# Doubiiu/ToonCrafter

Measured on AMD Instinct MI355X. Metric: interpolated frames/sec, 512x320x16f DDIM-50, higher is better.
Workload: dtype bf16; 1 GPU; ToonCrafter_512 320x512x16f ddim_steps=50 CFG 7.5 bf16, 1 clip per GPU (BASELINE.json configs[1]); sampler + 16f decode + 14f re-decode + splice; a different clip every step; parallelism=dp1 (independent clips, one RCCL gather)

## Files before the change

tooncrafter_amd/csrc/attention.hip:

```cpp
#include "attn_tile64.h"
#include "gemm_common.h"

#include <stdlib.h>

namespace {

constexpr int KT = 64;
constexpr int K_STRIDE = 144;
constexpr int VT_STRIDE = 136;
constexpr int K_BYTES = KT * K_STRIDE;
constexpr int VT_BYTES = 64 * VT_STRIDE;

__global__ __launch_bounds__(256) void attn_d64_kernel(const TcAttnParams p) {
  __shared__ __attribute__((aligned(16))) char smem[K_BYTES + VT_BYTES];
  char* ks = smem;
  char* vts = smem + K_BYTES;

  const int tid = threadIdx.x, lane = tid & 63, wave = tid >> 6;
  const int l31 = lane & 31, half = lane >> 5;
  const int b = blockIdx.z, h = blockIdx.y;
  const int kvb = b / p.kv_bdiv;
  const bf16_t* qb = reinterpret_cast<const bf16_t*>(p.q) + (int64_t)b * p.q_sb + h * 64;
  const bf16_t* kb = reinterpret_cast<const bf16_t*>(p.k) + (int64_t)kvb * p.k_sb + h * 64;
  const bf16_t* vb = reinterpret_cast<const bf16_t*>(p.v) + (int64_t)kvb * p.v_sb + h * 64;
  bf16_t* ob = reinterpret_cast<bf16_t*>(p.o) + (int64_t)b * p.o_sb + h * 64;

  const int q_row = blockIdx.x * 128 + wave * 32 + l31;
  bf16x8 qf[4];
  tc_tile64_load_q(qf, qb, q_row, p.lq, p.q_ss, half);

  const float c = p.scale * 1.4426950408889634f;
  float m_run = -1e30f, l_run = 0.f;
  f32x16 oacc[2];
#pragma unroll
  for (int d = 0; d < 2; ++d)
#pragma unroll
    for (int r = 0; r < 16; ++r) oacc[d][r] = 0.f;

  u32x4 kreg[2], vreg[2];
  const u32x4 zero4 = {0u, 0u, 0u, 0u};
  auto load_kv = [&](int kt) {
    const int key0 = kt * KT;
#pragma unroll
    for (int it = 0; it < 2; ++it) {
      const int idx = tid + it * 256;
      const int key = idx & 63, dch = idx >> 6;
      const int gk = key0 + key;
      const int gkc = gk < p.lk ? gk : p.lk - 1;
      kreg[it] = *reinterpret_cast<const u32x4*>(kb + (int64_t)gkc * p.k_ss + dch * 8);
      vreg[it] = *reinterpret_cast<const u32x4*>(vb + (int64_t)gkc * p.v_ss + dch * 8);
    }
  };
  auto store_kv = [&](int kt) {
    const int key0 = kt * KT;
    uint16_t* vt = reinterpret_cast<uint16_t*>(vts);
#pragma unroll
    for (int it = 0; it < 2; ++it) {
      const int idx = tid + it * 256;
      const int key = idx & 63, dch = idx >> 6;
      const bool ok = key0 + key < p.lk;
      const u32x4 kv4 = ok ? kreg[it] : zero4;
      const u32x4 vv4 = ok ? vreg[it] : zero4;
      *reinterpret_cast<u32x4*>(ks + key * K_STRIDE + dch * 16) = kv4;
#pragma unroll
      for (int e = 0; e < 4; ++e) {
        vt[(dch * 8 + 2 * e) * (VT_STRIDE / 2) + key] = (uint16_t)(vv4[e] & 0xffffu);
        vt[(dch * 8 + 2 * e + 1) * (VT_STRIDE / 2) + key] = (uint16_t)(vv4[e] >> 16);
      }
    }
  };

  const int n_tiles = (p.lk + KT - 1) / KT;
  load_kv(0);
  for (int kt = 0; kt < n_tiles; ++kt) {
    const int key0 = kt * KT;
    __syncthreads();
    store_kv(kt);
    __syncthreads();
    if (kt + 1 < n_tiles) load_kv(kt + 1);

    f32x16 st[2];
    const f32x16 zero16 = {0.f, 0.f, 0.f, 0.f, 0.f, 0.f, 0.f, 0.f, 0.f, 0.f, 0.f, 0.f, 0.f, 0.f, 0.f, 0.f};
#pragma unroll
    for (int kbk = 0; kbk < 2; ++kbk) {
#pragma unroll
      for (int kk = 0; kk < 4; ++kk) {
        const bf16x8 kf = *reinterpret_cast<const bf16x8*>(ks + (kbk * 32 + l31) * K_STRIDE + kk * 32 + half * 16);
        st[kbk] = __builtin_amdgcn_mfma_f32_32x32x16_bf16(kf, qf[kk], kk == 0 ? zero16 : st[kbk], 0, 0, 0);
      }
    }
    tc_tile64_mask(st, key0, p.lk, half, -1e30f);
    tc_tile64_softmax(st, c, m_run, l_run, oacc);

#pragma unroll
    for (int kbk = 0; kbk < 2; ++kbk)
#pragma unroll
      for (int s = 0; s < 2; ++s) {
        const bf16x8 pf = tc_tile64_pack_p(st[kbk], s);
#pragma unroll
        for (int d = 0; d < 2; ++d) {
          const char* vrow = vts + (d * 32 + l31) * VT_STRIDE + (kbk * 32 + 16 * s + 4 * half) * 2;
          const u32x2 lo = *reinterpret_cast<const u32x2*>(vrow);
          const u32x2 hi = *reinterpret_cast<const u32x2*>(vrow + 16);
          u32x4 vv = {lo[0], lo[1], hi[0], hi[1]};
          oacc[d] = __builtin_amdgcn_mfma_f32_32x32x16_bf16(__builtin_bit_cast(bf16x8, vv), pf, oacc[d], 0, 0, 0);
        }
      }
  }

  if (q_row < p.lq) tc_tile64_store(oacc, l_run, ob + (int64_t)q_row * p.o_ss, half, p.accumulate);
}

constexpr int KD_TILE = KT * 128;
constexpr int DMA_STAGE = 2 * KD_TILE;

__device__ __forceinline__ u32x2 lds_read_tr16_b64(const char* p) {
  typedef short s16x4 __attribute__((ext_vector_type(4)));
  const s16x4 v = __builtin_amdgcn_ds_read_tr16_b64_v4i16((__attribute__((address_space(3))) s16x4*)(p));
  return __builtin_bit_cast(u32x2, v);
}

template <bool DUAL>
__global__ __launch_bounds__(256) void attn_d64_dma_kernel(const TcAttnParams p) {
  __shared__ __attribute__((aligned(1024))) char smem[2 * DMA_STAGE];

  const int tid = threadIdx.x, lane = tid & 63, wave = tid >> 6;
  const int wave_u = __builtin_amdgcn_readfirstlane(wave);
  const int l31 = lane & 31, half = lane >> 5;
  const int b = blockIdx.z, h = blockIdx.y;
  const bf16_t* qb = reinterpret_cast<const bf16_t*>(p.q) + (int64_t)b * p.q_sb + h * 64;
  bf16_t* ob = reinterpret_cast<bf16_t*>(p.o) + (int64_t)b * p.o_sb + h * 64;

  const int q_row = blockIdx.x * 128 + wave * 32 + l31;
  bf16x8 qf[4];
  tc_tile64_load_q(qf, qb, q_row, p.lq, p.q_ss, half);

  int k_off[4];
#pragma unroll
  for (int kk = 0; kk < 4; ++kk) k_off[kk] = l31 * 128 + (((kk * 2 + half) ^ ((l31 >> 1) & 7)) << 4);
  const int lg = lane & 15;
  int v_off[2];
#pragma unroll
  for (int d0 = 0; d0 < 2; ++d0) {
    const int vrow = lg >> 2;
    const int col = d0 * 32 + 16 * ((lane >> 4) & 1) + 4 * (lg & 3);
    const int chunk = (col >> 3) ^ (((vrow >> 1) & 1) << 2);
    v_off[d0] = vrow * 128 + chunk * 16 + (col & 7) * 2;
  }

  const float c = p.scale * 1.4426950408889634f;
  float m_run = -1e30f, l_run = 0.f;
  f32x16 oacc[2];
#pragma unroll
  for (int d = 0; d < 2; ++d)
#pragma unroll
    for (int r = 0; r < 16; ++r) oacc[d][r] = 0.f;
  const int prow = lane >> 3;

  auto run_stream = [&](const bf16_t* kb, const bf16_t* vb, const int lk, const int k_ss, const int v_ss) {
    const tc_rsrc_t k_rsrc = make_rsrc(kb, ((int64_t)(lk - 1) * k_ss + 64) * 2);
    const tc_rsrc_t v_rsrc = make_rsrc(vb, ((int64_t)(lk - 1) * v_ss + 64) * 2);
    uint32_t k_voff[2], v_voff[2];
    int piece_row[2];
#pragma unroll
    for (int i = 0; i < 2; ++i) {
      const int row = (wave + 4 * i) * 8 + prow;
      piece_row[i] = row;
      const int kchunk = (lane & 7) ^ ((row >> 1) & 7);
      const int vchunk = (lane & 7) ^ (((row >> 1) & 1) << 2);
      k_voff[i] = (uint32_t)(row * k_ss * 2 + kchunk * 16);
      v_voff[i] = (uint32_t)(row * v_ss * 2 + vchunk * 16);
    }
    auto dma_tile = [&](int kt, int stage) {
      const int key0 = kt * KT;
      char* sk = smem + stage * DMA_STAGE + wave_u * 1024;
      char* sv = sk + KD_TILE;
#pragma unroll
      for (int i = 0; i < 2; ++i) {
        const uint32_t dead = (key0 + piece_row[i] < lk) ? 0u : TC_OOB;
        glds16(k_rsrc, sk + i * 4096, k_voff[i] | dead, (uint32_t)key0 * (uint32_t)k_ss * 2u);
        glds16(v_rsrc, sv + i * 4096, v_voff[i] | dead, (uint32_t)key0 * (uint32_t)v_ss * 2u);
      }
    };

    const int n_tiles = (lk + KT - 1) / KT;
    dma_tile(0, 0);
    for (int kt = 0; kt < n_tiles; ++kt) {
      const int key0 = kt * KT;
      asm volatile("s_waitcnt vmcnt(0)" ::: "memory");
      __syncthreads();
      if (kt + 1 < n_tiles) dma_tile(kt + 1, (kt + 1) & 1);
      const char* ks = smem + (kt & 1) * DMA_STAGE;
      const char* vs = ks + KD_TILE;

      f32x16 st[2];
      const f32x16 zero16 = {0.f, 0.f, 0.f, 0.f, 0.f, 0.f, 0.f, 0.f, 0.f, 0.f, 0.f, 0.f, 0.f, 0.f, 0.f, 0.f};
#pragma unroll
      for (int kbk = 0; kbk < 2; ++kbk) {
#pragma unroll
        for (int kk = 0; kk < 4; ++kk) {
          const bf16x8 kf = *reinterpret_cast<const bf16x8*>(ks + kbk * 32 * 128 + k_off[kk]);
          st[kbk] = __builtin_amdgcn_mfma_f32_32x32x16_bf16(kf, qf[kk], kk == 0 ? zero16 : st[kbk], 0, 0, 0);
        }
      }
      tc_tile64_mask(st, key0, lk, half, -1e30f);
      tc_tile64_softmax(st, c, m_run, l_run, oacc);

#pragma unroll
      for (int kbk = 0; kbk < 2; ++kbk)
#pragma unroll
        for (int s = 0; s < 2; ++s) {
          const bf16x8 pf = tc_tile64_pack_p(st[kbk], s);
          const int kbase = (kbk * 32 + 16 * s + 4 * half) * 128;
#pragma unroll
          for (int d = 0; d < 2; ++d) {
            const u32x2 lo = lds_read_tr16_b64(vs + kbase + v_off[d]);
            const u32x2 hi = lds_read_tr16_b64(vs + kbase + 8 * 128 + v_off[d]);
            u32x4 vv = {lo[0], lo[1], hi[0], hi[1]};
            oacc[d] = __builtin_amdgcn_mfma_f32_32x32x16_bf16(__builtin_bit_cast(bf16x8, vv), pf, oacc[d], 0, 0, 0);
          }
        }
    }
  };

  {
    const int kvb = b / p.kv_bdiv;
    run_stream(reinterpret_cast<const bf16_t*>(p.k) + (int64_t)kvb * p.k_sb + h * 64,
               reinterpret_cast<const bf16_t*>(p.v) + (int64_t)kvb * p.v_sb + h * 64, p.lk, p.k_ss, p.v_ss);
  }
  f32x16 o1[2];
  if (DUAL) {
    const float inv1 = 1.0f / l_run;
#pragma unroll
    for (int d = 0; d < 2; ++d)
#pragma unroll
      for (int r = 0; r < 16; ++r) { o1[d][r] = oacc[d][r] * inv1; oacc[d][r] = 0.f; }
    m_run = -1e30f;
    l_run = 0.f;
    __syncthreads();
    const int kvb2 = b / p.kv2_bdiv;
    run_stream(reinterpret_cast<const bf16_t*>(p.k2) + (int64_t)kvb2 * p.k2_sb + h * 64,
               reinterpret_cast<const bf16_t*>(p.v2) + (int64_t)kvb2 * p.v2_sb + h * 64, p.lk2, p.k2_ss, p.v2_ss);
  }

  if (q_row < p.lq) tc_tile64_store<DUAL>(oacc, o1, l_run, ob + (int64_t)q_row * p.o_ss, half, p.accumulate);
}

__global__ __launch_bounds__(256) void attn_temporal_kernel(const bf16_t* __restrict__ qkv, bf16_t* __restrict__ out,
                                                           int nb, int t_len, int hw, int heads, float scale) {
  __shared__ float kv_s[4][2][16][64 + 4];
  const int lane = threadIdx.x & 63, wave = threadIdx.x >> 6;
  const int64_t seq = (int64_t)blockIdx.x * 4 + wave;
  const int64_t total = (int64_t)nb * hw * heads;
  const bool active = seq < total;
  const int64_t sq = active ? seq : total - 1;
  const int hd = (int)(sq % heads);
  const int64_t bp = sq / heads;
  const int px = (int)(bp % hw);
  const int bb = (int)(bp / hw);
  const int C = heads * 64;
  const int ld = 3 * C;
  const int64_t row0 = ((int64_t)bb * t_len) * hw + px;

#pragma unroll
  for (int it = 0; it < 2; ++it) {
    const int idx = lane + it * 64;
    const int fr = idx >> 3, ch = idx & 7;
    float kf[8], vf[8];
    if (fr < t_len) {
      const bf16_t* rp = qkv + (row0 + (int64_t)fr * hw) * ld + hd * 64 + ch * 8;
      unpack8(*reinterpret_cast<const u32x4*>(rp + C), kf);
      unpack8(*reinterpret_cast<const u32x4*>(rp + 2 * C), vf);
    } else {
#pragma unroll
      for (int e = 0; e < 8; ++e) { kf[e] = 0.f; vf[e] = 0.f; }
    }
#pragma unroll
// ... 38 lines not shown
#pragma unroll
  for (int j = 0; j < 16; ++j) {
    const float pj = s[j] * inv;
#pragma unroll
    for (int e = 0; e < 16; ++e) o[e] += pj * kv_s[wave][1][j][quarter * 16 + e];
  }
  if (active && qi < t_len) {
    bf16_t* op = out + (row0 + (int64_t)qi * hw) * C + hd * 64 + quarter * 16;
    *reinterpret_cast<u32x4*>(op) = pack8(o);
    *reinterpret_cast<u32x4*>(op + 8) = pack8(o + 8);
  }
}

}

extern "C" int tc_attn_d64(const TcAttnParams* pp, void* stream) {
  if (!pp) return TC_EINVAL;
  const TcAttnParams& p = *pp;
  if (!p.q || !p.k || !p.v || !p.o) return TC_EINVAL;
  if (p.batch <= 0 || p.heads <= 0 || p.lq <= 0 || p.lk <= 0 || p.kv_bdiv <= 0) return TC_EINVAL;
  if (!tc_tile64_aligned(p.q, p.q_ss, p.q_sb) || !tc_tile64_aligned(p.k, p.k_ss, p.k_sb) ||
      !tc_tile64_aligned(p.v, p.v_ss, p.v_sb) || !tc_tile64_aligned(p.o, p.o_ss, p.o_sb))
    return TC_EALIGN;
  if (p.heads > 65535 || p.batch > 65535) return TC_ESHAPE;
  const bool dual = p.k2 != nullptr;
  if (dual) {
    if (!p.v2 || p.lk2 <= 0 || p.kv2_bdiv <= 0) return TC_EINVAL;
    if (!tc_tile64_aligned(p.k2, p.k2_ss, p.k2_sb) || !tc_tile64_aligned(p.v2, p.v2_ss, p.v2_sb)) return TC_EALIGN;
  }
  dim3 grid((p.lq + 127) / 128, p.heads, p.batch), block(256);
  static const bool use_reg = [] { const char* e = getenv("TC_ATTN_STAGE"); return e && e[0] == 'r'; }();
  const bool fits = (int64_t)p.lk * p.k_ss * 2 < 0x7fffff00LL && (int64_t)p.lk * p.v_ss * 2 < 0x7fffff00LL &&
                    p.k_ss >= 64 && p.v_ss >= 64;
  if (dual) {
    const bool fits2 = (int64_t)p.lk2 * p.k2_ss * 2 < 0x7fffff00LL && (int64_t)p.lk2 * p.v2_ss * 2 < 0x7fffff00LL &&
                       p.k2_ss >= 64 && p.v2_ss >= 64;
    if (!fits || !fits2) return TC_ESHAPE;
    hipLaunchKernelGGL(attn_d64_dma_kernel<true>, grid, block, 0, reinterpret_cast<hipStream_t>(stream), p);
  } else if (!use_reg && fits) {
    hipLaunchKernelGGL(attn_d64_dma_kernel<false>, grid, block, 0, reinterpret_cast<hipStream_t>(stream), p);
  } else {
    hipLaunchKernelGGL(attn_d64_kernel, grid, block, 0, reinterpret_cast<hipStream_t>(stream), p);
  }
  TC_LAUNCH_CHECK();
  return TC_OK;
}

extern "C" int tc_attn_temporal(const tc_bf16* qkv, tc_bf16* out, int32_t b, int32_t t, int32_t hw,
                                int32_t heads, float scale, void* stream) {
  if (!qkv || !out || b <= 0 || t <= 0 || hw <= 0 || heads <= 0) return TC_EINVAL;
  if (t > TC_TEMPORAL_MAX_FRAMES) return TC_ESHAPE;
  if (!tc_aligned16(qkv) || !tc_aligned16(out)) return TC_EALIGN;
  if (t > 16)
    return attn_temporal_long_launch(reinterpret_cast<const bf16_t*>(qkv), reinterpret_cast<bf16_t*>(out), b, t, hw, heads,
                                     scale, reinterpret_cast<hipStream_t>(stream));
  const int64_t total = (int64_t)b * hw * heads;
  const int64_t nblk = (total + 3) / 4;
  if (nblk > 0x7fffffffLL) return TC_ESHAPE;
  hipLaunchKernelGGL(attn_temporal_kernel, dim3((unsigned)nblk), dim3(256), 0, reinterpret_cast<hipStream_t>(stream),
                     reinterpret_cast<const bf16_t*>(qkv), reinterpret_cast<bf16_t*>(out), b, t, hw, heads, scale);
  TC_LAUNCH_CHECK();
  return TC_OK;
}
```

tooncrafter_amd/csrc/attn_tile64.h:

```cpp
#pragma once
#include "common.h"

namespace {

__device__ __forceinline__ void tc_tile64_load_q(bf16x8 (&qf)[4], const bf16_t* qb, int q_row, int lq, int q_ss, int half) {
  const int q_ld = q_row < lq ? q_row : lq - 1;
#pragma unroll
  for (int kk = 0; kk < 4; ++kk) qf[kk] = *reinterpret_cast<const bf16x8*>(qb + (int64_t)q_ld * q_ss + kk * 16 + half * 8);
}

template <class S>
__device__ __forceinline__ void tc_tile64_mask(S (&s)[2], int key0, int lk, int half, float masked) {
  if (key0 + 64 <= lk) return;
#pragma unroll
  for (int kbk = 0; kbk < 2; ++kbk)
#pragma unroll
    for (int r = 0; r < 16; ++r) {
      const int key = key0 + kbk * 32 + (r & 3) + 8 * (r >> 2) + 4 * half;
      s[kbk][r] = key < lk ? s[kbk][r] : masked;
    }
}

__device__ __forceinline__ void tc_tile64_raise_max(float m_new, float& m_run, float& l_run, f32x16 (&oacc)[2]) {
  if (!__all(m_new == m_run)) {
// ... 5 lines not shown
      for (int r = 0; r < 16; ++r) oacc[d][r] *= alpha;
    m_run = m_new;
  }
}

__device__ __forceinline__ void tc_tile64_softmax(f32x16 (&st)[2], float c, float& m_run, float& l_run, f32x16 (&oacc)[2]) {
  float mx = st[0][0];
#pragma unroll
  for (int kbk = 0; kbk < 2; ++kbk)
#pragma unroll
    for (int r = 0; r < 16; ++r) mx = fmaxf(mx, st[kbk][r]);
  mx = fmaxf(mx, __shfl_xor(mx, 32, 64));
  tc_tile64_raise_max(fmaxf(m_run, mx * c), m_run, l_run, oacc);
  float rs = 0.f;
#pragma unroll
  for (int kbk = 0; kbk < 2; ++kbk)
#pragma unroll
    for (int r = 0; r < 16; ++r) {
      const float pv = fast_exp2(fmaf(st[kbk][r], c, -m_run));
      st[kbk][r] = pv;
      rs += pv;
    }
  rs += __shfl_xor(rs, 32, 64);
  l_run += rs;
}

__device__ __forceinline__ bf16x8 tc_tile64_pack_p(const f32x16& st, int s) {
  bf16x8 pf;
#pragma unroll
  for (int j = 0; j < 8; ++j) pf[j] = (bf16_t)st[8 * s + j];
  return pf;
}

template <bool DUAL>
__device__ __forceinline__ void tc_tile64_store(const f32x16 (&oacc)[2], const f32x16 (&o1)[2], float l_run, bf16_t* orow,
                                                int half, bool accumulate) {
  const float inv = 1.0f / l_run;
#pragma unroll
  for (int d = 0; d < 2; ++d)
#pragma unroll
    for (int g = 0; g < 4; ++g) {
      float x0 = oacc[d][4 * g + 0] * inv, x1 = oacc[d][4 * g + 1] * inv;
      float x2 = oacc[d][4 * g + 2] * inv, x3 = oacc[d][4 * g + 3] * inv;
      if (DUAL) { x0 += o1[d][4 * g + 0]; x1 += o1[d][4 * g + 1]; x2 += o1[d][4 * g + 2]; x3 += o1[d][4 * g + 3]; }
      u32x2* dst = reinterpret_cast<u32x2*>(orow + d * 32 + 8 * g + 4 * half);
      if (accumulate) {
        const u32x2 old = *dst;
        x0 += __uint_as_float(old[0] << 16);
        x1 += __uint_as_float(old[0] & 0xffff0000u);
        x2 += __uint_as_float(old[1] << 16);
        x3 += __uint_as_float(old[1] & 0xffff0000u);
      }
      const u32x2 out = {pack2(x0, x1), pack2(x2, x3)};
      *dst = out;
    }
}
__device__ __forceinline__ void tc_tile64_store(const f32x16 (&oacc)[2], float l_run, bf16_t* orow, int half, bool accumulate) {
  tc_tile64_store<false>(oacc,  oacc, l_run, orow, half, accumulate);
}

inline bool tc_tile64_aligned(const void* p, int64_t ss, int64_t sb) { return tc_aligned16(p) && !(ss & 7) && !(sb & 7); }

}
```

tooncrafter_amd/csrc/gemm_epilogue.h:

```cpp
#pragma once
#include "gemm_common.h"

template <bool PLAIN>
__device__ __forceinline__ void epi_geglu_pair(const TcGemmParams& p, float* x, const float* gt, const float* bv, const float* bg) {
#if defined(TC_ABLATE) && (TC_ABLATE & 8)
  if (PLAIN) { x[0] = (x[0] + bv[0]) * (gt[0] + bg[0]); x[1] = (x[1] + bv[1]) * (gt[1] + bg[1]); }
#else
  if (PLAIN) {
    const tc_f32x2 v = {x[0] + bv[0], x[1] + bv[1]};
    const tc_f32x2 h = v * gelu_erf_f2(tc_f32x2{gt[0] + bg[0], gt[1] + bg[1]});
    x[0] = h[0]; x[1] = h[1];
  }
#endif
  else {
    const tc_f32x2 v = {x[0] * p.alpha + bv[0], x[1] * p.alpha + bv[1]};
    const tc_f32x2 h = v * gelu_erf_f2(tc_f32x2{gt[0] * p.alpha + bg[0], gt[1] * p.alpha + bg[1]}) * p.out_scale;
    x[0] = h[0]; x[1] = h[1];
  }
}

template <class Stored>
__device__ __forceinline__ void epi_finish_row8(const TcGemmParams& p, char* c_base, const bf16_t* res_base, int m, int n0,
                                                float (&x)[8], Stored&& stored) {
  float bv[8] = {0.f, 0.f, 0.f, 0.f, 0.f, 0.f, 0.f, 0.f};
// ... 37 lines not shown
__device__ __forceinline__ void epi_slab_pass16(const TcGemmParams& p, float* slab, const f32x4 (&acc)[NT], int lane, int frow,
                                                int fq, int col_w0, char* c_base, const bf16_t* res_base, RowOf&& row_of,
                                                Stored&& stored) {
  constexpr int WT = 16 * NT, VPR = WT / 8;
#pragma unroll
  for (int j = 0; j < NT; ++j)
#pragma unroll
    for (int r = 0; r < 4; ++r) slab[(fq * 4 + r) * WT + j * 16 + frow] = acc[j][r];
#pragma unroll
  for (int q = 0; q < (16 * VPR + 63) / 64; ++q) {
    const int v = lane + 64 * q;
    const int lr = v / VPR, vc = v - lr * VPR;
    const int m = row_of(lr);
    const int n0 = col_w0 + vc * 8;
    if (v < 16 * VPR && m < p.m && n0 < p.n) {
      const f32x4 lo = *reinterpret_cast<const f32x4*>(slab + lr * WT + vc * 8);
      const f32x4 hi = *reinterpret_cast<const f32x4*>(slab + lr * WT + vc * 8 + 4);
      float x[8] = {lo[0], lo[1], lo[2], lo[3], hi[0], hi[1], hi[2], hi[3]};
      epi_finish_row8(p, c_base, res_base, m, n0, x, [&](const u32x4& packed) { stored(q, packed); });
    }
  }
}

template <int HALF, int NJ, int LD>
__device__ __forceinline__ void epi_spill32_half(float* slab, const f32x16* acc, int frow, int fhalf) {
#pragma unroll
  for (int j = 0; j < NJ; ++j)
#pragma unroll
    for (int q = 0; q < 8; ++q) {
      const int r = 8 * HALF + q;
      const int lr = (r & 3) + 4 * fhalf + 8 * ((r >> 2) & 1);
      slab[lr * LD + j * 32 + frow] = acc[j][r];
    }
}

template <int HALF, int NJ, class RowOf>
__device__ __forceinline__ void epi_fused_out_pass(float* slab, const f32x16* acc, int lane, int n0w, const float* bias,
                                                   const bf16_t* x, int ldx, bf16_t* out, int ldo, RowOf&& row_of) {
  epi_spill32_half<HALF, NJ, 64>(slab, acc, lane & 31, lane >> 5);
  const int vc = lane & 7, lr0 = lane >> 3;
  const int n0 = n0w + vc * 8;
  if (vc * 8 < NJ * 32) {
#pragma unroll
    for (int qq = 0; qq < 2; ++qq) {
      const int lr = lr0 + 8 * qq;
      int64_t m;
      const bool ok = row_of(lr, m);
      const f32x4 lo = *reinterpret_cast<const f32x4*>(slab + lr * 64 + vc * 8);
      const f32x4 hi = *reinterpret_cast<const f32x4*>(slab + lr * 64 + vc * 8 + 4);
      if (ok) {
        float xv[8] = {lo[0], lo[1], lo[2], lo[3], hi[0], hi[1], hi[2], hi[3]};
        float rf[8];
        unpack8(*reinterpret_cast<const u32x4*>(x + m * ldx + n0), rf);
#pragma unroll
        for (int e = 0; e < 8; ++e) xv[e] = (xv[e] + bias[n0 + e]) + rf[e];
        *reinterpret_cast<u32x4*>(out + m * ldo + n0) = pack8(xv);
      }
    }
  }
}

template <bool GEGLU, int BM, int BN>
struct EpiGeo {
  static constexpr int GROUPS = GEGLU ? BN / 16 : BN / 8;
  static constexpr int ITERS = BM * GROUPS / 256;
  static constexpr int ROWS_PER_IT = 256 / GROUPS;
// ... 172 lines not shown
```

tooncrafter_amd/csrc/gemm_wide.hip:

```cpp
#include "gemm_epilogue.h"

namespace {

constexpr int WBM = TC_BIG;
constexpr int WTHREADS = 512;

template <int GATHER, int TNW, bool PIPE>
__global__ __launch_bounds__(WTHREADS, 2) void gemm_wide_kernel(const TcGemmParams p, const int order) {
  constexpr int BN = 64 * TNW;
  constexpr int WN = 32 * TNW;
  constexpr int STAGE_BYTES = (WBM + BN) * TC_BK * 2;
  constexpr int RA = WBM / 64, RB = BN / 64;
  constexpr int SLAB_FLOATS = 16 * WN;
  static_assert(8 * SLAB_FLOATS * 4 <= 2 * STAGE_BYTES, "epilogue slabs must fit in the pipeline buffers");
  __shared__ __attribute__((aligned(1024))) char smem[2 * STAGE_BYTES];

  const int tid = threadIdx.x;
  const int lane = tid & 63;
  const int wave = tid >> 6;
  const int wm = wave >> 1, wn = wave & 1;
  const int wave_u = __builtin_amdgcn_readfirstlane(wave);

  const int tiles_n = (p.n + BN - 1) / BN;
  const int tiles_m = (p.m + WBM - 1) / WBM;
  int tile_m, tile_n;
  tc_tile_of_block(blockIdx.x, tiles_m, tiles_n, order, tile_m, tile_n);
  if (tile_m >= tiles_m) return;

  const int64_t bz = blockIdx.z;
  const tc_rsrc_t w_rsrc = make_rsrc(reinterpret_cast<const bf16_t*>(p.w) + bz * p.stride_w, tc_w_extent(p));

  const int lrow = tid >> 3;
  const int chunk = (tid & 7) ^ ((lrow >> 1) & 7);
  AGather<GATHER, RA> ag;
  ag.init(p, tile_m * WBM, lrow, 64, chunk);
  const tc_rsrc_t a_rsrc = tc_a_rsrc(p, bz, ag.row_lo);
  uint32_t b_voff[RB];
#pragma unroll
  for (int i = 0; i < RB; ++i) {
    const int n = tile_n * BN + lrow + 64 * i;
    b_voff[i] = n < p.n ? (uint32_t)((int64_t)n * p.ldw * 2 + chunk * 16) : TC_OOB;
  }
  const bool k_ragged = (p.k & (TC_BK - 1)) != 0;

  auto load_tile = [&](int kb, int stage) {
    const int k0 = kb * TC_BK;
    uint32_t a_voff[RA], a_soff;
    ag.offsets(p, k0, chunk, a_voff, a_soff);
    const uint32_t kill = (k_ragged && (k0 + chunk * 8 >= p.k)) ? TC_OOB : 0u;
    char* sa = smem + stage * STAGE_BYTES + wave_u * 1024;
    char* sb = sa + WBM * TC_BK * 2;
#pragma unroll
    for (int i = 0; i < RB; ++i) glds16(w_rsrc, sb + i * 8192, b_voff[i] | kill, (uint32_t)k0 * 2u);
#pragma unroll
    for (int i = 0; i < RA; ++i) glds16(a_rsrc, sa + i * 8192, a_voff[i] | kill, a_soff);
  };

  f32x16 acc[2][TNW];
#pragma unroll
  for (int i = 0; i < 2; ++i)
#pragma unroll
    for (int j = 0; j < TNW; ++j)
#pragma unroll
      for (int r = 0; r < 16; ++r) acc[i][j][r] = 0.f;

  const int frow = lane & 31;
  const int fhalf = lane >> 5;

  auto compute = [&](int stage) {
    const char* sa = smem + stage * STAGE_BYTES;
    const char* sb = sa + WBM * TC_BK * 2;
    auto frags = [&](int kk, bf16x8 (&a)[2], bf16x8 (&b)[TNW]) {
      const int c = kk * 2 + fhalf;
#pragma unroll
      for (int i = 0; i < 2; ++i)
        a[i] = *reinterpret_cast<const bf16x8*>(sa + lds_off(wm * 64 + i * 32 + frow, c));
#pragma unroll
      for (int j = 0; j < TNW; ++j)
        b[j] = *reinterpret_cast<const bf16x8*>(sb + lds_off(wn * WN + j * 32 + frow, c));
    };
    auto mfmas = [&](bf16x8 (&a)[2], bf16x8 (&b)[TNW]) {
#pragma unroll
      for (int j = 0; j < TNW; ++j)
#pragma unroll
        for (int i = 0; i < 2; ++i)
          acc[i][j] = __builtin_amdgcn_mfma_f32_32x32x16_bf16(a[i], b[j], acc[i][j], 0, 0, 0);
    };
    if constexpr (TNW <= 4) {
      bf16x8 af[2][2], bf[2][TNW];
      frags(0, af[0], bf[0]);
      frags(1, af[1], bf[1]);
      __builtin_amdgcn_sched_barrier(0);
      mfmas(af[0], bf[0]);
      __builtin_amdgcn_sched_barrier(0);
      frags(2, af[0], bf[0]);
      __builtin_amdgcn_sched_barrier(0);
      mfmas(af[1], bf[1]);
      __builtin_amdgcn_sched_barrier(0);
      frags(3, af[1], bf[1]);
      __builtin_amdgcn_sched_barrier(0);
      mfmas(af[0], bf[0]);
      mfmas(af[1], bf[1]);
      __builtin_amdgcn_sched_barrier(0);
    } else {
#pragma unroll
      for (int kk = 0; kk < 4; ++kk) {
        bf16x8 af[2], bf[TNW];
        frags(kk, af, bf);
        mfmas(af, bf);
      }
    }
  };

  const int nk = (p.k + TC_BK - 1) / TC_BK;
  if (PIPE) tc_kloop_pipe<RA + RB>(0, nk, load_tile, compute);
  else tc_kloop_plain(0, nk, load_tile, compute);

  const bool geglu = p.act == TC_ACT_GEGLU;
  const int n_out = geglu ? p.n / 2 : p.n;
  float* slab = reinterpret_cast<float*>(smem) + wave * SLAB_FLOATS;
  const bf16_t* res_base = p.residual ? reinterpret_cast<const bf16_t*>(p.residual) + bz * p.stride_c : nullptr;
  char* c_base = reinterpret_cast<char*>(p.c) + bz * p.stride_c * (p.out_f32 ? 4 : 2);
  const int col_w0 = tile_n * BN + wn * WN;

  auto epi_pass = [&](auto I_, auto H_) {
    constexpr int i = decltype(I_)::value, half = decltype(H_)::value;
    epi_spill32_half<half, TNW, WN>(slab, acc[i], frow, fhalf);
    const int row_base = tile_m * WBM + wm * 64 + i * 32 + half * 16;
    if (!geglu) {
      constexpr int VPR = WN / 8;
      constexpr int NV = 16 * VPR / 64;
#pragma unroll
      for (int q = 0; q < NV; ++q) {
        const int v = lane + 64 * q;
        const int lr = v / VPR, vc = v - lr * VPR;
        const int m = row_base + lr;
        const int n0 = col_w0 + vc * 8;
        const f32x4 lo = *reinterpret_cast<const f32x4*>(slab + lr * WN + vc * 8);
        const f32x4 hi = *reinterpret_cast<const f32x4*>(slab + lr * WN + vc * 8 + 4);
        if (m < p.m && n0 < p.n) {
          float x[8] = {lo[0], lo[1], lo[2], lo[3], hi[0], hi[1], hi[2], hi[3]};
          epi_finish_row8(p, c_base, res_base, m, n0, x);
        }
      }
    } else {
      constexpr int VPR = WN / 16;
      constexpr int TOT = 16 * VPR;
#pragma unroll
      for (int q = 0; q < (TOT + 63) / 64; ++q) {
        const int v = lane + 64 * q;
        const int lr = v / VPR, u = v - lr * VPR;
        const int m = row_base + lr;
        const int pc = 32 * (u >> 1) + 8 * (u & 1);
        const int n0 = (col_w0 >> 1) + u * 8;
        if (v < TOT && m < p.m && n0 < n_out) {
          const f32x4 lo = *reinterpret_cast<const f32x4*>(slab + lr * WN + pc);
          const f32x4 hi = *reinterpret_cast<const f32x4*>(slab + lr * WN + pc + 4);
          const f32x4 glo = *reinterpret_cast<const f32x4*>(slab + lr * WN + pc + 16);
          const f32x4 ghi = *reinterpret_cast<const f32x4*>(slab + lr * WN + pc + 20);
          float x[8] = {lo[0], lo[1], lo[2], lo[3], hi[0], hi[1], hi[2], hi[3]};
          float gt[8] = {glo[0], glo[1], glo[2], glo[3], ghi[0], ghi[1], ghi[2], ghi[3]};
          float bv[8] = {0.f, 0.f, 0.f, 0.f, 0.f, 0.f, 0.f, 0.f}, bg[8] = {0.f, 0.f, 0.f, 0.f, 0.f, 0.f, 0.f, 0.f};
          if (p.bias) {
            const float* bp = p.bias + col_w0 + pc;
            const f32x4 b0 = *reinterpret_cast<const f32x4*>(bp), b1 = *reinterpret_cast<const f32x4*>(bp + 4);
            const f32x4 g0 = *reinterpret_cast<const f32x4*>(bp + 16), g1 = *reinterpret_cast<const f32x4*>(bp + 20);
#pragma unroll
            for (int e = 0; e < 4; ++e) { bv[e] = b0[e]; bv[4 + e] = b1[e]; bg[e] = g0[e]; bg[4 + e] = g1[e]; }
          }
#pragma unroll
          for (int e = 0; e < 8; e += 2) epi_geglu_pair<false>(p, x + e, gt + e, bv + e, bg + e);
          if (p.out_f32) {
            float* op = reinterpret_cast<float*>(c_base) + (int64_t)m * p.ldc + n0;
            *reinterpret_cast<f32x4*>(op) = f32x4{x[0], x[1], x[2], x[3]};
            *reinterpret_cast<f32x4*>(op + 4) = f32x4{x[4], x[5], x[6], x[7]};
          } else {
            *reinterpret_cast<u32x4*>(reinterpret_cast<bf16_t*>(c_base) + (int64_t)m * p.ldc + n0) = pack8(x);
          }
        }
      }
    }
  };
  using std::integral_constant;
  epi_pass(integral_constant<int, 0>{}, integral_constant<int, 0>{});
  epi_pass(integral_constant<int, 0>{}, integral_constant<int, 1>{});
  epi_pass(integral_constant<int, 1>{}, integral_constant<int, 0>{});
  epi_pass(integral_constant<int, 1>{}, integral_constant<int, 1>{});
}

}

void tc_gemm_wide_launch(const TcGemmParams& p, const TcGemmRoute& r, hipStream_t s) {
  const dim3 grid(r.grid[0], r.grid[1], r.grid[2]), block(r.block);
  const auto go = [&](auto g, auto t) {
    constexpr int G = decltype(g)::value, TNW = decltype(t)::value;
    if (r.pipe) hipLaunchKernelGGL((gemm_wide_kernel<G, TNW, true>), grid, block, 0, s, p, r.order);
    else hipLaunchKernelGGL((gemm_wide_kernel<G, TNW, false>), grid, block, 0, s, p, r.order);
  };
  tc_with_gather(p.gather, [&](auto g) {
    if (r.tnw == 5) go(g, std::integral_constant<int, 5>{});
    else if (r.tnw == 4) go(g, std::integral_constant<int, 4>{});
    else go(g, std::integral_constant<int, 2>{});
  });
}
```

tooncrafter_amd/csrc/mfma_shape.h:

```cpp
#pragma once
#include <stdlib.h>

constexpr int TC_GEMM_MFMA_DEFAULT = 16;
constexpr int TC_QKV_MFMA_DEFAULT = 16;

inline int tc_mfma_shape(const char* name, int dflt) {
  const char* e = getenv(name);
  const int v = e ? atoi(e) : dflt;
  return v == 16 || v == 32 ? v : dflt;
}
inline int tc_gemm_mfma() { return tc_mfma_shape("TC_GEMM_MFMA", TC_GEMM_MFMA_DEFAULT); }
inline int tc_qkv_mfma() { return tc_mfma_shape("TC_QKV_MFMA", TC_QKV_MFMA_DEFAULT); }
```

Measured before the change: 8.277 frames/s.

## Add 16x16x32 MFMA paths to wide GEMM and d64 attention kernels

Adds a 16x16x32 bf16 MFMA variant of the wide GEMM kernel, with per-TNW LDS fragment scheduling and a padded epilogue slab. The wide GEMM now follows the existing GEMM MFMA-shape setting, which defaults to 16. It also adds templated 16x16 variants of the register-staged and DMA d64 attention kernels, with new softmax, mask and store helpers; attention stays on the 32x32 shape by default. The aim is better issue interleaving and occupancy from smaller MFMA tiles. The cost is more LDS fragment reads per MFMA and more accumulator bookkeeping.

```diff
diff --git a/tooncrafter_amd/csrc/attention.hip b/tooncrafter_amd/csrc/attention.hip
--- a/tooncrafter_amd/csrc/attention.hip
+++ b/tooncrafter_amd/csrc/attention.hip
@@ -1,5 +1,6 @@
 #include "attn_tile64.h"
 #include "gemm_common.h"
+#include "mfma_shape.h"
 
 #include <stdlib.h>
 
@@ -11,6 +12,7 @@
 constexpr int K_BYTES = KT * K_STRIDE;
 constexpr int VT_BYTES = 64 * VT_STRIDE;
 
+template <int MF>
 __global__ __launch_bounds__(256) void attn_d64_kernel(const TcAttnParams p) {
   __shared__ __attribute__((aligned(16))) char smem[K_BYTES + VT_BYTES];
   char* ks = smem;
@@ -25,9 +27,11 @@
   const bf16_t* vb = reinterpret_cast<const bf16_t*>(p.v) + (int64_t)kvb * p.v_sb + h * 64;
   bf16_t* ob = reinterpret_cast<bf16_t*>(p.o) + (int64_t)b * p.o_sb + h * 64;
 
-  const int q_row = blockIdx.x * 128 + wave * 32 + l31;
-  bf16x8 qf[4];
-  tc_tile64_load_q(qf, qb, q_row, p.lq, p.q_ss, half);
+  const int l15 = lane & 15, fq = lane >> 4;
+  const int q_row = blockIdx.x * 128 + wave * 32 + (MF == 16 ? l15 : l31);
+  bf16x8 qf[4], qf16[2][2];
+  if constexpr (MF == 16) tc_tile64_load_q16(qf16, qb, q_row, p.lq, p.q_ss, fq);
+  else tc_tile64_load_q(qf, qb, q_row, p.lq, p.q_ss, half);
 
   const float c = p.scale * 1.4426950408889634f;
   float m_run = -1e30f, l_run = 0.f;
@@ -36,6 +40,12 @@
   for (int d = 0; d < 2; ++d)
 #pragma unroll
     for (int r = 0; r < 16; ++r) oacc[d][r] = 0.f;
+  float m_run16[2] = {-1e30f, -1e30f}, l_run16[2] = {0.f, 0.f};
+  f32x4 oacc16[2][4];
+#pragma unroll
+  for (int b2 = 0; b2 < 2; ++b2)
+#pragma unroll
+    for (int dt = 0; dt < 4; ++dt) oacc16[b2][dt] = f32x4{0.f, 0.f, 0.f, 0.f};
 
   u32x4 kreg[2], vreg[2];
   const u32x4 zero4 = {0u, 0u, 0u, 0u};
@@ -79,6 +89,37 @@
     __syncthreads();
     if (kt + 1 < n_tiles) load_kv(kt + 1);
 
+    if constexpr (MF == 16) {
+      f32x4 st[2][4];
+      const f32x4 zero4f = {0.f, 0.f, 0.f, 0.f};
+#pragma unroll
+      for (int t = 0; t < 4; ++t)
+#pragma unroll
+        for (int s2 = 0; s2 < 2; ++s2) {
+          const bf16x8 kf = *reinterpret_cast<const bf16x8*>(ks + (t * 16 + l15) * K_STRIDE + s2 * 64 + fq * 16);
+#pragma unroll
+          for (int b2 = 0; b2 < 2; ++b2)
+            st[b2][t] = __builtin_amdgcn_mfma_f32_16x16x32_bf16(kf, qf16[b2][s2], s2 == 0 ? zero4f : st[b2][t], 0, 0, 0);
+        }
+      tc_tile64_mask16(st, key0, p.lk, fq, -1e30f);
+      tc_tile64_softmax16(st, c, m_run16, l_run16, oacc16);
+#pragma unroll
+      for (int s = 0; s < 2; ++s) {
+        const bf16x8 pf[2] = {tc_tile64_pack_p16(st[0], s), tc_tile64_pack_p16(st[1], s)};
+#pragma unroll
+        for (int dt = 0; dt < 4; ++dt) {
+          const char* vrow = vts + (dt * 16 + l15) * VT_STRIDE + (32 * s + 4 * fq) * 2;
+          const u32x2 lo = *reinterpret_cast<const u32x2*>(vrow);
+          const u32x2 hi = *reinterpret_cast<const u32x2*>(vrow + 32);
+          const u32x4 vv = {lo[0], lo[1], hi[0], hi[1]};
+#pragma unroll
+          for (int b2 = 0; b2 < 2; ++b2)
+            oacc16[b2][dt] = __builtin_amdgcn_mfma_f32_16x16x32_bf16(__builtin_bit_cast(bf16x8, vv), pf[b2], oacc16[b2][dt], 0, 0, 0);
+        }
+      }
+      continue;
+    }
+
     f32x16 st[2];
     const f32x16 zero16 = {0.f, 0.f, 0.f, 0.f, 0.f, 0.f, 0.f, 0.f, 0.f, 0.f, 0.f, 0.f, 0.f, 0.f, 0.f, 0.f};
 #pragma unroll
@@ -108,6 +149,13 @@
       }
   }
 
+  if constexpr (MF == 16) {
+#pragma unroll
+    for (int b2 = 0; b2 < 2; ++b2)
+      if (q_row + 16 * b2 < p.lq)
+        tc_tile64_store16<false>(oacc16[b2], oacc16[b2], l_run16[b2], ob + (int64_t)(q_row + 16 * b2) * p.o_ss, fq, p.accumulate);
+    return;
+  }
   if (q_row < p.lq) tc_tile64_store(oacc, l_run, ob + (int64_t)q_row * p.o_ss, half, p.accumulate);
 }
 
@@ -120,7 +168,7 @@
   return __builtin_bit_cast(u32x2, v);
 }
 
-template <bool DUAL>
+template <bool DUAL, int MF = 32>
 __global__ __launch_bounds__(256) void attn_d64_dma_kernel(const TcAttnParams p) {
   __shared__ __attribute__((aligned(1024))) char smem[2 * DMA_STAGE];
 
@@ -131,9 +179,11 @@
   const bf16_t* qb = reinterpret_cast<const bf16_t*>(p.q) + (int64_t)b * p.q_sb + h * 64;
   bf16_t* ob = reinterpret_cast<bf16_t*>(p.o) + (int64_t)b * p.o_sb + h * 64;
 
-  const int q_row = blockIdx.x * 128 + wave * 32 + l31;
-  bf16x8 qf[4];
-  tc_tile64_load_q(qf, qb, q_row, p.lq, p.q_ss, half);
+  const int l15 = lane & 15, fq = lane >> 4;
+  const int q_row = blockIdx.x * 128 + wave * 32 + (MF == 16 ? l15 : l31);
+  bf16x8 qf[4], qf16[2][2];
+  if constexpr (MF == 16) tc_tile64_load_q16(qf16, qb, q_row, p.lq, p.q_ss, fq);
+  else tc_tile64_load_q(qf, qb, q_row, p.lq, p.q_ss, half);
 
   int k_off[4];
 #pragma unroll
@@ -147,6 +197,16 @@
     const int chunk = (col >> 3) ^ (((vrow >> 1) & 1) << 2);
     v_off[d0] = vrow * 128 + chunk * 16 + (col & 7) * 2;
   }
+  int k_off16[2], v_off16[4];
+#pragma unroll
+  for (int ks = 0; ks < 2; ++ks) k_off16[ks] = l15 * 128 + (((ks * 4 + fq) ^ ((l15 >> 1) & 7)) << 4);
+#pragma unroll
+  for (int dt = 0; dt < 4; ++dt) {
+    const int vrow = lg >> 2;
+    const int col = dt * 16 + 4 * (lg & 3);
+    const int chunk = (col >> 3) ^ (((vrow >> 1) & 1) << 2);
+    v_off16[dt] = vrow * 128 + chunk * 16 + (col & 7) * 2;
+  }
 
   const float c = p.scale * 1.4426950408889634f;
   float m_run = -1e30f, l_run = 0.f;
@@ -155,6 +215,12 @@
   for (int d = 0; d < 2; ++d)
 #pragma unroll
     for (int r = 0; r < 16; ++r) oacc[d][r] = 0.f;
+  float m_run16[2] = {-1e30f, -1e30f}, l_run16[2] = {0.f, 0.f};
+  f32x4 oacc16[2][4];
+#pragma unroll
+  for (int b2 = 0; b2 < 2; ++b2)
+#pragma unroll
+    for (int dt = 0; dt < 4; ++dt) oacc16[b2][dt] = f32x4{0.f, 0.f, 0.f, 0.f};
   const int prow = lane >> 3;
 
   auto run_stream = [&](const bf16_t* kb, const bf16_t* vb, const int lk, const int k_ss, const int v_ss) {
@@ -193,6 +259,37 @@
       const char* ks = smem + (kt & 1) * DMA_STAGE;
       const char* vs = ks + KD_TILE;
 
+      if constexpr (MF == 16) {
+        f32x4 st[2][4];
+        const f32x4 zero4f = {0.f, 0.f, 0.f, 0.f};
+#pragma unroll
+        for (int t = 0; t < 4; ++t)
+#pragma unroll
+          for (int s2 = 0; s2 < 2; ++s2) {
+            const bf16x8 kf = *reinterpret_cast<const bf16x8*>(ks + t * 16 * 128 + k_off16[s2]);
+#pragma unroll
+            for (int b2 = 0; b2 < 2; ++b2)
+              st[b2][t] = __builtin_amdgcn_mfma_f32_16x16x32_bf16(kf, qf16[b2][s2], s2 == 0 ? zero4f : st[b2][t], 0, 0, 0);
+          }
+        tc_tile64_mask16(st, key0, lk, fq, -1e30f);
+        tc_tile64_softmax16(st, c, m_run16, l_run16, oacc16);
+#pragma unroll
+        for (int s = 0; s < 2; ++s) {
+          const bf16x8 pf[2] = {tc_tile64_pack_p16(st[0], s), tc_tile64_pack_p16(st[1], s)};
+          const int kbase = (32 * s + 4 * fq) * 128;
+#pragma unroll
+          for (int dt = 0; dt < 4; ++dt) {
+            const u32x2 lo = lds_read_tr16_b64(vs + kbase + v_off16[dt]);
+            const u32x2 hi = lds_read_tr16_b64(vs + kbase + 16 * 128 + v_off16[dt]);
+            const u32x4 vv = {lo[0], lo[1], hi[0], hi[1]};
+#pragma unroll
+            for (int b2 = 0; b2 < 2; ++b2)
+              oacc16[b2][dt] = __builtin_amdgcn_mfma_f32_16x16x32_bf16(__builtin_bit_cast(bf16x8, vv), pf[b2], oacc16[b2][dt], 0, 0, 0);
+          }
+        }
+        continue;
+      }
+
       f32x16 st[2];
       const f32x16 zero16 = {0.f, 0.f, 0.f, 0.f, 0.f, 0.f, 0.f, 0.f, 0.f, 0.f, 0.f, 0.f, 0.f, 0.f, 0.f, 0.f};
 #pragma unroll
@@ -229,7 +326,18 @@
                reinterpret_cast<const bf16_t*>(p.v) + (int64_t)kvb * p.v_sb + h * 64, p.lk, p.k_ss, p.v_ss);
   }
   f32x16 o1[2];
+  f32x4 o116[2][4];
   if (DUAL) {
+    if constexpr (MF == 16) {
+#pragma unroll
+      for (int b2 = 0; b2 < 2; ++b2) {
+        const float inv1 = 1.0f / l_run16[b2];
+#pragma unroll
+        for (int dt = 0; dt < 4; ++dt) { o116[b2][dt] = oacc16[b2][dt] * inv1; oacc16[b2][dt] = f32x4{0.f, 0.f, 0.f, 0.f}; }
+        m_run16[b2] = -1e30f;
+        l_run16[b2] = 0.f;
+      }
+    } else {
     const float inv1 = 1.0f / l_run;
 #pragma unroll
     for (int d = 0; d < 2; ++d)
@@ -237,12 +345,20 @@
       for (int r = 0; r < 16; ++r) { o1[d][r] = oacc[d][r] * inv1; oacc[d][r] = 0.f; }
     m_run = -1e30f;
     l_run = 0.f;
+    }
     __syncthreads();
     const int kvb2 = b / p.kv2_bdiv;
     run_stream(reinterpret_cast<const bf16_t*>(p.k2) + (int64_t)kvb2 * p.k2_sb + h * 64,
                reinterpret_cast<const bf16_t*>(p.v2) + (int64_t)kvb2 * p.v2_sb + h * 64, p.lk2, p.k2_ss, p.v2_ss);
   }
 
+  if constexpr (MF == 16) {
+#pragma unroll
+    for (int b2 = 0; b2 < 2; ++b2)
+      if (q_row + 16 * b2 < p.lq)
+        tc_tile64_store16<DUAL>(oacc16[b2], o116[b2], l_run16[b2], ob + (int64_t)(q_row + 16 * b2) * p.o_ss, fq, p.accumulate);
+    return;
+  }
   if (q_row < p.lq) tc_tile64_store<DUAL>(oacc, o1, l_run, ob + (int64_t)q_row * p.o_ss, half, p.accumulate);
 }
 
@@ -347,15 +463,20 @@
   static const bool use_reg = [] { const char* e = getenv("TC_ATTN_STAGE"); return e && e[0] == 'r'; }();
   const bool fits = (int64_t)p.lk * p.k_ss * 2 < 0x7fffff00LL && (int64_t)p.lk * p.v_ss * 2 < 0x7fffff00LL &&
                     p.k_ss >= 64 && p.v_ss >= 64;
+  const bool mf16 = tc_attn_mfma() == 16;
+  const hipStream_t st = reinterpret_cast<hipStream_t>(stream);
   if (dual) {
     const bool fits2 = (int64_t)p.lk2 * p.k2_ss * 2 < 0x7fffff00LL && (int64_t)p.lk2 * p.v2_ss * 2 < 0x7fffff00LL &&
                        p.k2_ss >= 64 && p.v2_ss >= 64;
     if (!fits || !fits2) return TC_ESHAPE;
-    hipLaunchKernelGGL(attn_d64_dma_kernel<true>, grid, block, 0, reinterpret_cast<hipStream_t>(stream), p);
+    if (mf16) hipLaunchKernelGGL((attn_d64_dma_kernel<true, 16>), grid, block, 0, st, p);
+    else hipLaunchKernelGGL((attn_d64_dma_kernel<true, 32>), grid, block, 0, st, p);
   } else if (!use_reg && fits) {
-    hipLaunchKernelGGL(attn_d64_dma_kernel<false>, grid, block, 0, reinterpret_cast<hipStream_t>(stream), p);
+    if (mf16) hipLaunchKernelGGL((attn_d64_dma_kernel<false, 16>), grid, block, 0, st, p);
+    else hipLaunchKernelGGL((attn_d64_dma_kernel<false, 32>), grid, block, 0, st, p);
   } else {
-    hipLaunchKernelGGL(attn_d64_kernel, grid, block, 0, reinterpret_cast<hipStream_t>(stream), p);
+    if (mf16) hipLaunchKernelGGL(attn_d64_kernel<16>, grid, block, 0, st, p);
+    else hipLaunchKernelGGL(attn_d64_kernel<32>, grid, block, 0, st, p);
   }
   TC_LAUNCH_CHECK();
   return TC_OK;
diff --git a/tooncrafter_amd/csrc/attn_tile64.h b/tooncrafter_amd/csrc/attn_tile64.h
--- a/tooncrafter_amd/csrc/attn_tile64.h
+++ b/tooncrafter_amd/csrc/attn_tile64.h
@@ -61,6 +61,19 @@
   return pf;
 }
 
+__device__ __forceinline__ void tc_tile64_put4(bf16_t* at, float x0, float x1, float x2, float x3, bool accumulate) {
+  u32x2* dst = reinterpret_cast<u32x2*>(at);
+  if (accumulate) {
+    const u32x2 old = *dst;
+    x0 += __uint_as_float(old[0] << 16);
+    x1 += __uint_as_float(old[0] & 0xffff0000u);
+    x2 += __uint_as_float(old[1] << 16);
+    x3 += __uint_as_float(old[1] & 0xffff0000u);
+  }
+  const u32x2 out = {pack2(x0, x1), pack2(x2, x3)};
+  *dst = out;
+}
+
 template <bool DUAL>
 __device__ __forceinline__ void tc_tile64_store(const f32x16 (&oacc)[2], const f32x16 (&o1)[2], float l_run, bf16_t* orow,
                                                 int half, bool accumulate) {
@@ -72,22 +85,94 @@
       float x0 = oacc[d][4 * g + 0] * inv, x1 = oacc[d][4 * g + 1] * inv;
       float x2 = oacc[d][4 * g + 2] * inv, x3 = oacc[d][4 * g + 3] * inv;
       if (DUAL) { x0 += o1[d][4 * g + 0]; x1 += o1[d][4 * g + 1]; x2 += o1[d][4 * g + 2]; x3 += o1[d][4 * g + 3]; }
-      u32x2* dst = reinterpret_cast<u32x2*>(orow + d * 32 + 8 * g + 4 * half);
-      if (accumulate) {
-        const u32x2 old = *dst;
-        x0 += __uint_as_float(old[0] << 16);
-        x1 += __uint_as_float(old[0] & 0xffff0000u);
-        x2 += __uint_as_float(old[1] << 16);
-        x3 += __uint_as_float(old[1] & 0xffff0000u);
-      }
-      const u32x2 out = {pack2(x0, x1), pack2(x2, x3)};
-      *dst = out;
+      tc_tile64_put4(orow + d * 32 + 8 * g + 4 * half, x0, x1, x2, x3, accumulate);
     }
 }
 __device__ __forceinline__ void tc_tile64_store(const f32x16 (&oacc)[2], float l_run, bf16_t* orow, int half, bool accumulate) {
   tc_tile64_store<false>(oacc,  oacc, l_run, orow, half, accumulate);
 }
 
+
+__device__ __forceinline__ void tc_tile64_load_q16(bf16x8 (&qf)[2][2], const bf16_t* qb, int q_row0, int lq, int q_ss, int fq) {
+#pragma unroll
+  for (int b = 0; b < 2; ++b) {
+    const int q_row = q_row0 + 16 * b;
+    const int q_ld = q_row < lq ? q_row : lq - 1;
+#pragma unroll
+    for (int ks = 0; ks < 2; ++ks) qf[b][ks] = *reinterpret_cast<const bf16x8*>(qb + (int64_t)q_ld * q_ss + ks * 32 + fq * 8);
+  }
+}
+
+__device__ __forceinline__ void tc_tile64_mask16(f32x4 (&s)[2][4], int key0, int lk, int fq, float masked) {
+  if (key0 + 64 <= lk) return;
+#pragma unroll
+  for (int kt = 0; kt < 4; ++kt)
+#pragma unroll
+    for (int r = 0; r < 4; ++r) {
+      const bool ok = key0 + kt * 16 + 4 * fq + r < lk;
+#pragma unroll
+      for (int b = 0; b < 2; ++b) s[b][kt][r] = ok ? s[b][kt][r] : masked;
+    }
+}
+
+__device__ __forceinline__ void tc_tile64_softmax16(f32x4 (&st)[2][4], float c, float (&m_run)[2], float (&l_run)[2],
+                                                    f32x4 (&oacc)[2][4]) {
+  float m_new[2];
+#pragma unroll
+  for (int b = 0; b < 2; ++b) {
+    float mx = st[b][0][0];
+#pragma unroll
+    for (int kt = 0; kt < 4; ++kt)
+#pragma unroll
+      for (int r = 0; r < 4; ++r) mx = fmaxf(mx, st[b][kt][r]);
+    m_new[b] = fmaxf(m_run[b], tc_max_rows(mx) * c);
+  }
+  if (!__all(m_new[0] == m_run[0] && m_new[1] == m_run[1])) {
+#pragma unroll
+    for (int b = 0; b < 2; ++b) {
+      const float alpha = fast_exp2(m_run[b] - m_new[b]);
+      l_run[b] *= alpha;
+#pragma unroll
+      for (int dt = 0; dt < 4; ++dt)
+#pragma unroll
+        for (int r = 0; r < 4; ++r) oacc[b][dt][r] *= alpha;
+      m_run[b] = m_new[b];
+    }
+  }
+#pragma unroll
+  for (int b = 0; b < 2; ++b) {
+    float rs = 0.f;
+#pragma unroll
+    for (int kt = 0; kt < 4; ++kt)
+#pragma unroll
+      for (int r = 0; r < 4; ++r) {
+        const float pv = fast_exp2(fmaf(st[b][kt][r], c, -m_run[b]));
+        st[b][kt][r] = pv;
+        rs += pv;
+      }
+    l_run[b] += tc_sum_rows(rs);
+  }
+}
+
+__device__ __forceinline__ bf16x8 tc_tile64_pack_p16(const f32x4 (&st)[4], int s) {
+  bf16x8 pf;
+#pragma unroll
+  for (int j = 0; j < 8; ++j) pf[j] = (bf16_t)st[2 * s + (j >> 2)][j & 3];
+  return pf;
+}
+
+template <bool DUAL>
+__device__ __forceinline__ void tc_tile64_store16(const f32x4 (&oacc)[4], const f32x4 (&o1)[4], float l_run, bf16_t* orow, int fq,
+                                                  bool accumulate) {
+  const float inv = 1.0f / l_run;
+#pragma unroll
+  for (int dt = 0; dt < 4; ++dt) {
+    float x0 = oacc[dt][0] * inv, x1 = oacc[dt][1] * inv, x2 = oacc[dt][2] * inv, x3 = oacc[dt][3] * inv;
+    if (DUAL) { x0 += o1[dt][0]; x1 += o1[dt][1]; x2 += o1[dt][2]; x3 += o1[dt][3]; }
+    tc_tile64_put4(orow + dt * 16 + 4 * fq, x0, x1, x2, x3, accumulate);
+  }
+}
+
 inline bool tc_tile64_aligned(const void* p, int64_t ss, int64_t sb) { return tc_aligned16(p) && !(ss & 7) && !(sb & 7); }
 
 }
diff --git a/tooncrafter_amd/csrc/gemm_epilogue.h b/tooncrafter_amd/csrc/gemm_epilogue.h
--- a/tooncrafter_amd/csrc/gemm_epilogue.h
+++ b/tooncrafter_amd/csrc/gemm_epilogue.h
@@ -93,6 +93,14 @@
       const int lr = (r & 3) + 4 * fhalf + 8 * ((r >> 2) & 1);
       slab[lr * LD + j * 32 + frow] = acc[j][r];
     }
+}
+
+template <int NJ, int LD>
+__device__ __forceinline__ void epi_spill16_tile(float* slab, const f32x4* acc, int frow16, int fq) {
+#pragma unroll
+  for (int j = 0; j < NJ; ++j)
+#pragma unroll
+    for (int r = 0; r < 4; ++r) slab[(4 * fq + r) * LD + j * 16 + frow16] = acc[j][r];
 }
 
 template <int HALF, int NJ, class RowOf>
diff --git a/tooncrafter_amd/csrc/gemm_wide.hip b/tooncrafter_amd/csrc/gemm_wide.hip
--- a/tooncrafter_amd/csrc/gemm_wide.hip
+++ b/tooncrafter_amd/csrc/gemm_wide.hip
@@ -1,17 +1,19 @@
 #include "gemm_epilogue.h"
+#include "mfma_shape.h"
 
 namespace {
 
 constexpr int WBM = TC_BIG;
 constexpr int WTHREADS = 512;
 
-template <int GATHER, int TNW, bool PIPE>
+template <int GATHER, int TNW, bool PIPE, int MF = 32>
 __global__ __launch_bounds__(WTHREADS, 2) void gemm_wide_kernel(const TcGemmParams p, const int order) {
   constexpr int BN = 64 * TNW;
   constexpr int WN = 32 * TNW;
+  constexpr int SLD = MF == 16 ? WN + 4 : WN;
   constexpr int STAGE_BYTES = (WBM + BN) * TC_BK * 2;
   constexpr int RA = WBM / 64, RB = BN / 64;
-  constexpr int SLAB_FLOATS = 16 * WN;
+  constexpr int SLAB_FLOATS = 16 * SLD;
   static_assert(8 * SLAB_FLOATS * 4 <= 2 * STAGE_BYTES, "epilogue slabs must fit in the pipeline buffers");
   __shared__ __attribute__((aligned(1024))) char smem[2 * STAGE_BYTES];
 
@@ -63,13 +65,88 @@
     for (int j = 0; j < TNW; ++j)
 #pragma unroll
       for (int r = 0; r < 16; ++r) acc[i][j][r] = 0.f;
+  f32x4 acc16[4][2 * TNW];
+#pragma unroll
+  for (int i = 0; i < 4; ++i)
+#pragma unroll
+    for (int j = 0; j < 2 * TNW; ++j) acc16[i][j] = f32x4{0.f, 0.f, 0.f, 0.f};
 
   const int frow = lane & 31;
   const int fhalf = lane >> 5;
+  const int frow16 = lane & 15;
+  const int fq = lane >> 4;
 
   auto compute = [&](int stage) {
     const char* sa = smem + stage * STAGE_BYTES;
     const char* sb = sa + WBM * TC_BK * 2;
+    if constexpr (MF == 16) {
+      auto frags16 = [&](int ks, bf16x8 (&a)[4], bf16x8 (&b)[2 * TNW]) {
+        const int c = ks * 4 + fq;
+#pragma unroll
+        for (int i = 0; i < 4; ++i)
+          a[i] = *reinterpret_cast<const bf16x8*>(sa + lds_off(wm * 64 + i * 16 + frow16, c));
+#pragma unroll
+        for (int j = 0; j < 2 * TNW; ++j)
+          b[j] = *reinterpret_cast<const bf16x8*>(sb + lds_off(wn * WN + j * 16 + frow16, c));
+      };
+      auto mfmas16 = [&](bf16x8 (&a)[4], bf16x8 (&b)[2 * TNW]) {
+#pragma unroll
+        for (int j = 0; j < 2 * TNW; ++j)
+#pragma unroll
+          for (int i = 0; i < 4; ++i)
+            acc16[i][j] = __builtin_amdgcn_mfma_f32_16x16x32_bf16(a[i], b[j], acc16[i][j], 0, 0, 0);
+      };
+      if constexpr (TNW == 2) {
+        bf16x8 a16[2][4], b16[2][2 * TNW];
+        frags16(0, a16[0], b16[0]);
+        frags16(1, a16[1], b16[1]);
+        __builtin_amdgcn_sched_barrier(0);
+        mfmas16(a16[0], b16[0]);
+        mfmas16(a16[1], b16[1]);
+        __builtin_amdgcn_sched_barrier(0);
+      } else if constexpr (TNW == 4) {
+        bf16x8 a0[4], a1[4], bl[4], bh[4];
+        const int c0 = fq, c1 = 4 + fq;
+        auto rd_a = [&](int c, bf16x8 (&a)[4]) {
+#pragma unroll
+          for (int i = 0; i < 4; ++i) a[i] = *reinterpret_cast<const bf16x8*>(sa + lds_off(wm * 64 + i * 16 + frow16, c));
+        };
+        auto rd_b = [&](int c, int j0, bf16x8 (&b)[4]) {
+#pragma unroll
+          for (int j = 0; j < 4; ++j) b[j] = *reinterpret_cast<const bf16x8*>(sb + lds_off(wn * WN + (j0 + j) * 16 + frow16, c));
+        };
+        auto mm = [&](auto J0_, bf16x8 (&a)[4], bf16x8 (&b)[4]) {
+          constexpr int j0 = decltype(J0_)::value;
+#pragma unroll
+          for (int j = 0; j < 4; ++j)
+#pragma unroll
+            for (int i = 0; i < 4; ++i)
+              acc16[i][j0 + j] = __builtin_amdgcn_mfma_f32_16x16x32_bf16(a[i], b[j], acc16[i][j0 + j], 0, 0, 0);
+        };
+        using std::integral_constant;
+        rd_a(c0, a0); rd_b(c0, 0, bl); rd_b(c0, 4, bh); rd_a(c1, a1);
+        __builtin_amdgcn_sched_barrier(0);
+        mm(integral_constant<int, 0>{}, a0, bl);
+        __builtin_amdgcn_sched_barrier(0);
+        rd_b(c1, 0, bl);
+        __builtin_amdgcn_sched_barrier(0);
+        mm(integral_constant<int, 4>{}, a0, bh);
+        __builtin_amdgcn_sched_barrier(0);
+        rd_b(c1, 4, bh);
+        __builtin_amdgcn_sched_barrier(0);
+        mm(integral_constant<int, 0>{}, a1, bl);
+        mm(integral_constant<int, 4>{}, a1, bh);
+        __builtin_amdgcn_sched_barrier(0);
+      } else {
+#pragma unroll
+        for (int ks = 0; ks < 2; ++ks) {
+          bf16x8 a16[4], b16[2 * TNW];
+          frags16(ks, a16, b16);
+          mfmas16(a16, b16);
+        }
+      }
+      return;
+    }
     auto frags = [&](int kk, bf16x8 (&a)[2], bf16x8 (&b)[TNW]) {
       const int c = kk * 2 + fhalf;
 #pragma unroll
@@ -125,7 +202,8 @@
 
   auto epi_pass = [&](auto I_, auto H_) {
     constexpr int i = decltype(I_)::value, half = decltype(H_)::value;
-    epi_spill32_half<half, TNW, WN>(slab, acc[i], frow, fhalf);
+    if constexpr (MF == 16) epi_spill16_tile<2 * TNW, SLD>(slab, acc16[2 * i + half], frow16, fq);
+    else epi_spill32_half<half, TNW, WN>(slab, acc[i], frow, fhalf);
     const int row_base = tile_m * WBM + wm * 64 + i * 32 + half * 16;
     if (!geglu) {
       constexpr int VPR = WN / 8;
@@ -136,8 +214,8 @@
         const int lr = v / VPR, vc = v - lr * VPR;
         const int m = row_base + lr;
         const int n0 = col_w0 + vc * 8;
-        const f32x4 lo = *reinterpret_cast<const f32x4*>(slab + lr * WN + vc * 8);
-        const f32x4 hi = *reinterpret_cast<const f32x4*>(slab + lr * WN + vc * 8 + 4);
+        const f32x4 lo = *reinterpret_cast<const f32x4*>(slab + lr * SLD + vc * 8);
+        const f32x4 hi = *reinterpret_cast<const f32x4*>(slab + lr * SLD + vc * 8 + 4);
         if (m < p.m && n0 < p.n) {
           float x[8] = {lo[0], lo[1], lo[2], lo[3], hi[0], hi[1], hi[2], hi[3]};
           epi_finish_row8(p, c_base, res_base, m, n0, x);
@@ -154,10 +232,10 @@
         const int pc = 32 * (u >> 1) + 8 * (u & 1);
         const int n0 = (col_w0 >> 1) + u * 8;
         if (v < TOT && m < p.m && n0 < n_out) {
-          const f32x4 lo = *reinterpret_cast<const f32x4*>(slab + lr * WN + pc);
-          const f32x4 hi = *reinterpret_cast<const f32x4*>(slab + lr * WN + pc + 4);
-          const f32x4 glo = *reinterpret_cast<const f32x4*>(slab + lr * WN + pc + 16);
-          const f32x4 ghi = *reinterpret_cast<const f32x4*>(slab + lr * WN + pc + 20);
+          const f32x4 lo = *reinterpret_cast<const f32x4*>(slab + lr * SLD + pc);
+          const f32x4 hi = *reinterpret_cast<const f32x4*>(slab + lr * SLD + pc + 4);
+          const f32x4 glo = *reinterpret_cast<const f32x4*>(slab + lr * SLD + pc + 16);
+          const f32x4 ghi = *reinterpret_cast<const f32x4*>(slab + lr * SLD + pc + 20);
           float x[8] = {lo[0], lo[1], lo[2], lo[3], hi[0], hi[1], hi[2], hi[3]};
           float gt[8] = {glo[0], glo[1], glo[2], glo[3], ghi[0], ghi[1], ghi[2], ghi[3]};
           float bv[8] = {0.f, 0.f, 0.f, 0.f, 0.f, 0.f, 0.f, 0.f}, bg[8] = {0.f, 0.f, 0.f, 0.f, 0.f, 0.f, 0.f, 0.f};
@@ -192,10 +270,15 @@
 
 void tc_gemm_wide_launch(const TcGemmParams& p, const TcGemmRoute& r, hipStream_t s) {
   const dim3 grid(r.grid[0], r.grid[1], r.grid[2]), block(r.block);
+  const bool mf16 = tc_gemm_mfma() == 16;
   const auto go = [&](auto g, auto t) {
     constexpr int G = decltype(g)::value, TNW = decltype(t)::value;
-    if (r.pipe) hipLaunchKernelGGL((gemm_wide_kernel<G, TNW, true>), grid, block, 0, s, p, r.order);
-    else hipLaunchKernelGGL((gemm_wide_kernel<G, TNW, false>), grid, block, 0, s, p, r.order);
+    const auto with_mf = [&](auto mf) {
+      constexpr int MF = decltype(mf)::value;
+      if (r.pipe) hipLaunchKernelGGL((gemm_wide_kernel<G, TNW, true, MF>), grid, block, 0, s, p, r.order);
+      else hipLaunchKernelGGL((gemm_wide_kernel<G, TNW, false, MF>), grid, block, 0, s, p, r.order);
+    };
+    if (mf16) with_mf(std::integral_constant<int, 16>{}); else with_mf(std::integral_constant<int, 32>{});
   };
   tc_with_gather(p.gather, [&](auto g) {
     if (r.tnw == 5) go(g, std::integral_constant<int, 5>{});
diff --git a/tooncrafter_amd/csrc/mfma_shape.h b/tooncrafter_amd/csrc/mfma_shape.h
--- a/tooncrafter_amd/csrc/mfma_shape.h
+++ b/tooncrafter_amd/csrc/mfma_shape.h
@@ -3,6 +3,7 @@
 
 constexpr int TC_GEMM_MFMA_DEFAULT = 16;
 constexpr int TC_QKV_MFMA_DEFAULT = 16;
+constexpr int TC_ATTN_MFMA_DEFAULT = 32;
 
 inline int tc_mfma_shape(const char* name, int dflt) {
   const char* e = getenv(name);
@@ -10,4 +11,5 @@
   return v == 16 || v == 32 ? v : dflt;
 }
 inline int tc_gemm_mfma() { return tc_mfma_shape("TC_GEMM_MFMA", TC_GEMM_MFMA_DEFAULT); }
+inline int tc_attn_mfma() { return tc_mfma_shape("TC_ATTN_MFMA", TC_ATTN_MFMA_DEFAULT); }
 inline int tc_qkv_mfma() { return tc_mfma_shape("TC_QKV_MFMA", TC_QKV_MFMA_DEFAULT); }
```

Result: no change. 8.273 frames/s (-0.1%).
